# JohnGBaker/ptmcmc

Measured on AMD Instinct MI355X. Metric: ladder-wide MH steps/sec (D=32 Gaussian, 1024 temps), higher is better.
Workload: dtype f64

## Files before the change

### ptmcmc_amd/csrc/ptm_box_prefilter.hpp

```cpp
#pragma once
#include "ptm_kernels.hpp"

namespace ptm {

struct BoxPre {
  int W, Nt, r0, w_off;
  int rung0, nrung;
  int labelled;
  uint64_t seed, step;
  const double* x;
  const double *ll, *lp;
  const double* beta;
  const double* prop_tiles;
  const double* box_row;
  int* ntries;
  const int *pidx, *pcnt;
  int *cidx, *ccnt;
  unsigned long long* counts;
};

typedef double bp_d4 __attribute__((ext_vector_type(4)));
typedef double bp_d2 __attribute__((ext_vector_type(2)));

inline size_t box_prefilter_lds(int nrung) { return (size_t)(BM_TABLE_DOUBLES + 64) * sizeof(double) + ((size_t)nrung + 260) * sizeof(int); }

__global__ __launch_bounds__(256) void box_prefilter_kernel(const BoxPre p) {
  extern __shared__ __attribute__((aligned(16))) double bp_lds[];
  double* lbox = bp_lds + BM_TABLE_DOUBLES;
  int* tpre = reinterpret_cast<int*>(lbox + 64);
  const int wave = threadIdx.x >> 6, l = threadIdx.x & 63, q = l >> 4, j = l & 15;
#pragma unroll
  for (int t = 0; t < BM_TABLE_DOUBLES / 512; ++t)
    reinterpret_cast<bm_d2*>(bp_lds)[threadIdx.x + 256 * t] = reinterpret_cast<const bm_d2*>(BM_TABLE)[threadIdx.x + 256 * t];
  if (threadIdx.x < 64) lbox[threadIdx.x] = p.box_row[threadIdx.x];
  const int nrung = p.nrung, per = (nrung + 255) / 256;
  int loc = 0;
  for (int k = 0; k < per; ++k) {
    const int r = threadIdx.x * per + k;
    if (r < nrung) { loc += (p.pcnt[p.rung0 + r] + 255) >> 8; tpre[r] = loc; }
  }
  int* tsum = tpre + nrung;
  tsum[threadIdx.x] = loc;
  __syncthreads();
  if (threadIdx.x == 0) { int run = 0; for (int t = 0; t < 256; ++t) { const int v = tsum[t]; tsum[t] = run; run += v; } tsum[256] = run; }
  __syncthreads();
  const int off = tsum[threadIdx.x];
  for (int k = 0; k < per; ++k) {
    const int r = threadIdx.x * per + k;
    if (r < nrung) tpre[r] += off;
  }
  __syncthreads();
  const int ntiles = tsum[256];
  const bp_d2* box = reinterpret_cast<const bp_d2*>(lbox) + q;
  const int wmask = p.labelled ? 0xFFFF : -1;
  unsigned int seen = 0, settled = 0;
  for (int tile = blockIdx.x; tile < ntiles; tile += gridDim.x) {
    int lo = 0, hi = nrung - 1;
    while (lo < hi) { const int mid = (lo + hi) >> 1; if (tpre[mid] > tile) hi = mid; else lo = mid + 1; }
    const int r = __builtin_amdgcn_readfirstlane(lo);
    const int kb = tile - (r ? tpre[r - 1] : 0);
    const int rl = p.rung0 + r, rg = p.r0 + rl;
    const int start = (kb * 4 + wave) * 64, cnt = p.pcnt[rl];
    if (start >= cnt) continue;
    const int nact = cnt - start < 64 ? cnt - start : 64;
    const size_t lbase = (size_t)rl * p.W;
    const int mine = p.pidx[lbase + start + (l < nact ? l : nact - 1)];
    const int c = (int)lbase + (mine & wmask);
    const double ll = p.ll[c], lp = p.lp[c];
    const double beta = as_c(p.beta)[rg];
    const double* timg = p.prop_tiles + (size_t)rl * (16 * 64) + l;
    double ta[4];
#pragma unroll
    for (int sl = 0; sl < 4; ++sl) ta[sl] = timg[((0 * 4 + sl) * 2 + 0) * 64];
    const bp_d2 lo0 = box[0], lo1 = box[4], hi0 = box[16], hi1 = box[20];
    bp_d2 v0[4], v1[4];
    int wk[4];
#pragma unroll
    for (int g = 0; g < 4; ++g) {
      const int e = __shfl(mine, 16 * g + j, 64);
      const int slot = p.labelled ? (int)((unsigned int)e >> 16) : rl;
      wk[g] = e & wmask;
      const bp_d2* rp = reinterpret_cast<const bp_d2*>(p.x + ((size_t)slot * p.W + wk[g]) * 32) + q;
      v0[g] = rp[0];
      v1[g] = rp[4];
    }
    uint64_t inbox = 0;
#pragma unroll
    for (int g = 0; g < 4; ++g) {
      const uint32_t stream = (uint32_t)(wk[g] + p.w_off) * (uint32_t)p.Nt + (uint32_t)rg;
      const u32x4 o = draw_block(p.seed, TAG_MH, stream, p.step, (uint32_t)(1 + q));
      double z[4];
      boxmuller(o.v0, o.v1, (const double*)bp_lds, z[0], z[1]);
      boxmuller(o.v2, o.v3, (const double*)bp_lds, z[2], z[3]);
      bp_d4 acc = bp_d4{0.0, 0.0, 0.0, 0.0};
#pragma unroll
      for (int sl = 0; sl < 4; ++sl) acc = __builtin_amdgcn_mfma_f64_16x16x4f64(ta[sl], z[sl], acc, 0, 0, 0);
      const double x0 = v0[g].x + acc[0], x1 = v0[g].y + acc[1], x2 = v1[g].x + acc[2], x3 = v1[g].y + acc[3];
      const bool ok = !(x0 < lo0.x) & !(x0 > hi0.x) & !(x1 < lo0.y) & !(x1 > hi0.y) & !(x2 < lo1.x) & !(x2 > hi1.x) & !(x3 < lo1.y) & !(x3 > hi1.y);
      uint64_t b = __builtin_amdgcn_ballot_w64(ok);
      b &= b >> 32;
      b &= b >> 16;
      inbox |= (b & 0xFFFFull) << (16 * g);
    }
    const double cur_lpost = lp + beta * ll;
    const bool live = l < nact;
    const bool finite = __builtin_fabs(cur_lpost) < __builtin_inf();
    const bool settle = live && finite && ((inbox >> l) & 1ull) == 0;
    if (settle) p.ntries[c] += 1;
    const bool keep = live && !settle;
    const uint64_t kbits = __builtin_amdgcn_ballot_w64(keep);
    const int nk = __builtin_popcountll(kbits);
    int base = 0;
    if (l == 0 && nk) base = atomicAdd(&p.ccnt[rl], nk);
    base = __builtin_amdgcn_readfirstlane(base);
    if (keep) p.cidx[lbase + base + __builtin_popcountll(kbits & ((1ull << l) - 1ull))] = mine;
    seen += (unsigned int)nact;
    settled += (unsigned int)(nact - nk);
  }
  if (l == 0 && seen) {
    atomicAdd(p.counts, (unsigned long long)seen);
    if (settled) atomicAdd(p.counts + 1, (unsigned long long)settled);
  }
}

}
```

### ptmcmc_amd/csrc/ptm_engine.hip

```cpp
#include <hip/hip_runtime.h>

#include <algorithm>
#include <cmath>
#include <cstddef>
#include <cstdarg>
#include <cstdio>
#include <cstring>
#include <functional>
#include <memory>
#include <string>
#include <vector>

#include "../../include/ptm_engine.h"
#include "ptm_aux_kernels.hpp"
#include "ptm_box_prefilter.hpp"
#include "ptm_devlike_kernels.hpp"
#include "ptm_ess_kernels.hpp"
#include "ptm_evidence_kernels.hpp"
#include "ptm_launch.hpp"
#include "ptm_shard_rccl.hpp"

using namespace ptm;

static thread_local std::string g_err;
// ... 1145 lines not shown
  p.mix_K = e->mix_K; p.mix = e->mix;
  p.de_on = e->de_on ? 1 : 0; p.de_init_extra = e->de_init_extra; p.de_init = e->de_init; p.de_hast = e->de_hast; p.de_type = e->de_type;
  p.de_snooker = e->de.snooker; p.de_gamma_one = e->de.gamma_one_frac; p.de_gamma_div = e->de.reduce_gamma; p.de_ignore = e->de.ignore_frac;
  p.de_gamma_std = e->de_on ? 1.68 / std::sqrt((double)e->D) / e->de.reduce_gamma : 0.0;
  p.prior_k = e->prior_member + 1;
  p.betaC = e->betaC; p.beta_add = e->beta_add; p.beta_w = e->beta_w;
  p.x = labelled ? e->xdev : xrows(e); p.ll = e->ll; p.lp = e->lp;
  p.ntries = e->ntries; p.naccept = e->naccept; p.last_type = e->last_type; p.nhist = e->nhist;
  p.touch = e->touch; p.err = e->err;
  p.hist = e->hist;
  p.map = e->map;
  p.c_begin = 0; p.c_end = e->Nc;
  p.host_prop = e->pcb ? 1 : 0; p.hastings = e->hastings; p.htype = e->htype; p.hvalid = e->hvalid; p.acc_out = e->acc_out;
  return p;
}

static AdaArgs make_ada(const ptm_engine* e) {
  AdaArgs a;
  memset(&a, 0, sizeof a);
  if (!e->ada_on) return a;
  const size_t L = (size_t)e->ada.K + e->ada.K_inner, Nc = e->Nc;
  a.K = e->ada.K; a.nested = e->ada.nested; a.Ki = e->ada.K_inner; a.rate = e->ada.rate; a.rate_in = e->ada.rate_inner;
  a.leaf = e->ada_leaf; a.w = e->ada_dbl; a.th = e->ada_dbl + L * Nc; a.bits = e->ada_int; a.cnt = e->ada_int + 2 * Nc;
  return a;
}

const DpLaunch* ptm::dp_launch(int DP) {
  switch (DP) {
    case 4: return &dp_launch_4;
    case 8: return &dp_launch_8;
    case 16: return &dp_launch_16;
    case 32: return &dp_launch_32;
    case 64: return &dp_launch_64;
    case 128: return &dp_launch_128;
    case 256: return &dp_launch_256;
    case 512: return &dp_launch_512;
    case 1024: return &dp_launch_1024;
  }
  return nullptr;
}

static inline bool user_like(const ptm_engine* e) { return e->cb != nullptr || e->dfn != nullptr; }

static SweepPlan sweep_plan(const ptm_engine* e, long long chains, bool touched) {
  SweepFacts f;
  f.DP = e->DP; f.W = e->W; f.chains = chains; f.nloc = e->nloc;
  f.kind = e->prop_kind == PTM_PROP_DIAG ? PLAN_DIAG : (e->prop_kind == PTM_PROP_LOWER ? PLAN_LOWER : PLAN_DENSE);
  f.has_bounds = e->has_bounds; f.bounds_box = e->bounds_box; f.all_uniform = e->all_uniform; f.has_mean = e->has_mean; f.any_oned = e->any_oned;
  f.mix_K = e->mix_K;
  f.evolving = e->betaC != nullptr; f.tracked = e->hist.rungs || e->map.rungs;
  f.user_like = user_like(e); f.host_prop = e->pcb != nullptr; f.ada = e->ada_on;
  f.de = e->de_on || e->prior_member >= 0;
  f.mode = f.user_like ? 1 : 0;
  f.touched = touched;
  return plan_sweep(f, sweep_env());
}
static SweepPlan step_sweep_plan(const ptm_engine* e) { return sweep_plan(e, e->Nc, true); }

static bool lean_ev_sweeps(const ptm_engine* e) { return reads_ladder_major_beta(step_sweep_plan(e)); }

static int flush_nhist(ptm_engine* e) {
  if (!e->nhist_pending) return PTM_OK;
  hipLaunchKernelGGL(nhist_flush_kernel, dim3((unsigned)(((size_t)e->Nc + 255) / 256)), dim3(256), 0, e->stream, e->nhist, (size_t)e->Nc, e->nhist_pending);
  HIPCHK(hipGetLastError());
  e->nhist_pending = 0;
  return PTM_OK;
}

static bool row_labels_apply(const ptm_engine* e) {
  static const bool labels_ok = [] { const char* v = getenv("PTM_ROW_LABELS"); return !(v && *v == '0'); }();
  return labels_ok && e->nloc == e->Nt && !e->shard && e->W <= 65536 && e->Nt > 1 && step_sweep_plan(e).compacted;
}
static void flush_rows(ptm_engine* e) {
  e->rows_labelled = false;
  hipLaunchKernelGGL(restore_rows_kernel, dim3(e->W), dim3(256), (size_t)4 * e->nloc, e->stream, e->xdev, e->rowof, e->W, e->nloc, e->DP);
}

static int ensure_betaC(ptm_engine* e);
static int callback_host_part(ptm_engine* e) {
  const size_t Nc = e->Nc, DP = e->DP;
  HIPCHK(copy_unless_shared(e->h_xprop.data(), e->xprop, Nc * DP * 8 + Nc, hipMemcpyDeviceToHost, e->stream));
  HIPCHK(hipStreamSynchronize(e->stream));
  if (e->prior_cb) {
    std::vector<double> hll(Nc), hlp(Nc), hbeta(Nc), out;
    HIPCHK(hipMemcpy(hll.data(), e->ll, Nc * 8, hipMemcpyDeviceToHost));
    HIPCHK(hipMemcpy(hlp.data(), e->lp, Nc * 8, hipMemcpyDeviceToHost));
    { int rc2 = ensure_betaC(e); if (rc2) return rc2; }
    if (e->betaC) HIPCHK(hipMemcpy(hbeta.data(), e->betaC, Nc * 8, hipMemcpyDeviceToHost));
    std::vector<size_t> vp;
    for (size_t c = 0; c < Nc; ++c)
      if (e->h_gate[c] & 1) vp.push_back(c);
    int rcp = call_user_prior(e, e->h_xprop, vp, out);
    if (rcp) return rcp;
    std::vector<double> lpn(Nc, -__builtin_inf());
    for (size_t k = 0; k < vp.size(); ++k) {
      const size_t c = vp[k];
      const double beta = e->betaC ? hbeta[c] : e->h_beta[e->r0 + c / e->W];
      const double bl = beta * hll[c];
      const double cur_lpost = hlp[c] + bl;
      const double oldlprior = cur_lpost - bl;
      const double nl = out[k];
      lpn[c] = nl;
      const bool want = nl > -1e200 || nl - oldlprior > e->cfg.min_prior;
      e->h_gate[c] = (unsigned char)(1 | (want ? 2 : 0));
    }
    HIPCHK(hipMemcpyAsync(e->lprior_new, lpn.data(), Nc * 8, hipMemcpyHostToDevice, e->stream));
    HIPCHK(copy_unless_shared(e->gate, e->h_gate, Nc, hipMemcpyHostToDevice, e->stream));
    HIPCHK(hipStreamSynchronize(e->stream));
  }
  std::vector<size_t> pick;
  for (size_t c = 0; c < Nc; ++c)
    if (e->h_gate[c] & 2) pick.push_back(c);
  int rc = call_user(e, e->h_xprop, pick, e->h_llbatch);
  if (rc) return rc;
  for (size_t k = 0; k < pick.size(); ++k) e->h_llnew[pick[k]] = e->h_llbatch[k];
  HIPCHK(copy_unless_shared(e->llike_new, e->h_llnew.data(), Nc * 8, hipMemcpyHostToDevice, e->stream));
  return PTM_OK;
}

static int devlike_eval(ptm_engine* e, const unsigned char* gate, int gmask, int gval, const double* xsel, const double* xrest, double* dst,
                        unsigned char* gate_out, const double* lprior, bool best) {
  const int n = e->Nc, D = e->D;
  const int nchunk = (n + DL_CHUNK - 1) / DL_CHUNK;
  hipLaunchKernelGGL(devlike_count_kernel, dim3(nchunk), dim3(DL_CHUNK), 0, e->stream, n, gate, gmask, gval, e->dl_chunks);
  HIPCHK(hipGetLastError());
#define PTM_DL_PACK(N) case N: hipLaunchKernelGGL((devlike_pack_kernel<N>), dim3(nchunk), dim3(DL_CHUNK), 0, e->stream, n, D, nchunk, gate, gmask, gval, \
                                                  (const int*)e->dl_chunks, xsel, xrest, e->dl_x, e->dl_rows, e->dl_count); break;
  switch (e->DP) {
    PTM_DL_PACK(4) PTM_DL_PACK(8) PTM_DL_PACK(16) PTM_DL_PACK(32) PTM_DL_PACK(64) PTM_DL_PACK(128) PTM_DL_PACK(256) PTM_DL_PACK(512) PTM_DL_PACK(1024)
    default: return fail(PTM_ERR_UNSUPPORTED, "dim > 1024 is not built");
  }
#undef PTM_DL_PACK
  HIPCHK(hipGetLastError());
  if (!xrest) {
    const size_t tot = (size_t)n * D;
    hipLaunchKernelGGL(devlike_fill_kernel, dim3((unsigned)((tot + 255) / 256)), dim3(256), 0, e->stream, n, D, (const int32_t*)e->dl_count, e->dl_x);
    HIPCHK(hipGetLastError());
  }
  e->dfn(e->dfn_user, (void*)e->stream, n, D, e->dl_x, e->dl_count, e->dl_ll);
  hipLaunchKernelGGL(devlike_scatter_kernel, dim3(1), dim3(DL_SCATTER_THREADS), 0, e->stream, D, (const int32_t*)e->dl_count, (const int*)e->dl_rows,
                     (const double*)e->dl_ll, dst, gate_out, lprior, (const double*)e->dl_x, best ? e->dl_best : nullptr);
  HIPCHK(hipGetLastError());
  return PTM_OK;
}

static int devlike_reset_best(ptm_engine* e) {
  if (!e->dl_best) return PTM_OK;
  std::vector<double> b((size_t)e->D + 1, 0.0);
  b[0] = -__builtin_inf();
  return upload(e->dl_best, b.data(), b.size(), e->stream);
}

extern "C" int ptm_set_target_device(ptm_engine* e, ptm_loglike_device_fn fn, void* user, double* x_batch_dev, double* llike_batch_dev) {
  if (!e || !fn) return fail(PTM_ERR_INVALID, "null argument");
  SETTLE(e);
  NO_BATCH(e, "ptm_set_target_device");
  if (e->prior_cb) return fail(PTM_ERR_UNSUPPORTED, "a host-evaluated prior with a device likelihood is not built (ptm_set_prior_callback)");
  if (e->pcb) return fail(PTM_ERR_UNSUPPORTED, "host-side proposals with a device likelihood are not built (ptm_set_proposal_callback)");
  if (e->nloc != e->Nt) return fail(PTM_ERR_UNSUPPORTED, "a device likelihood on a rung shard is not built: split such a population by walkers");
  const size_t Nc = e->Nc, D = e->D, DP = e->DP;
  int rc;
  if (!e->dl_count &&
      ((rc = dalloc(&e->dl_count, 1)) || (rc = dalloc(&e->dl_rows, Nc)) || (rc = dalloc(&e->dl_chunks, (Nc + DL_CHUNK - 1) / DL_CHUNK)) ||
       (rc = dalloc(&e->dl_xprop, Nc * DP)) || (rc = dalloc(&e->dl_gate, Nc)) || (rc = dalloc(&e->dl_lprior_new, Nc)) ||
       (rc = dalloc(&e->dl_llike_new, Nc)) || (rc = dalloc(&e->dl_best, D + 1))))
    return rc;
  if (x_batch_dev) {
    if (e->dl_own_x && e->dl_x) { HIPCHK(hipStreamSynchronize(e->stream)); (void)hipFree(e->dl_x); }
    e->dl_x = x_batch_dev; e->dl_own_x = false;
  } else if (!e->dl_own_x) {
    e->dl_x = nullptr;
    if ((rc = dalloc(&e->dl_x, Nc * D))) return rc;
    e->dl_own_x = true;
  }
  if (llike_batch_dev) {
    if (e->dl_own_ll && e->dl_ll) { HIPCHK(hipStreamSynchronize(e->stream)); (void)hipFree(e->dl_ll); }
    e->dl_ll = llike_batch_dev; e->dl_own_ll = false;
  } else if (!e->dl_own_ll) {
    e->dl_ll = nullptr;
    if ((rc = dalloc(&e->dl_ll, Nc))) return rc;
    e->dl_own_ll = true;
  }
  HIPCHK(hipMemsetAsync(e->dl_gate, 0, Nc, e->stream));
  if ((rc = devlike_reset_best(e))) return rc;
  e->dfn = fn; e->dfn_user = user;
  e->cb = nullptr;
  e->have_target = 1;
  return PTM_OK;
}

extern "C" int ptm_target_device_rows(ptm_engine* e) {
  if (!e) return fail(PTM_ERR_INVALID, "null engine");
  return e->Nc;
}

extern "C" int ptm_get_best_evaluated(ptm_engine* e, double* lpost, double* x) {
  if (!e || !lpost) return fail(PTM_ERR_INVALID, "null argument");
  SETTLE(e);
  NO_BATCH(e, "ptm_get_best_evaluated");
  if (!e->dl_best) return fail(PTM_ERR_INVALID, "no device likelihood set (ptm_set_target_device)");
  std::vector<double> b((size_t)e->D + 1);
  HIPCHK(hipMemcpyAsync(b.data(), e->dl_best, b.size() * 8, hipMemcpyDeviceToHost, e->stream));
  HIPCHK(hipStreamSynchronize(e->stream));
  *lpost = b[0];
  if (x) memcpy(x, b.data() + 1, (size_t)e->D * 8);
  return PTM_OK;
}

static int devlike_debug(ptm_engine* e, const double* X, int n, double* llike) {
  const size_t Nc = e->Nc, D = e->D;
  std::vector<double> rows(Nc * D);
  for (size_t k0 = 0; k0 < (size_t)n; k0 += Nc) {
    const size_t m = std::min(Nc, (size_t)n - k0);
    for (size_t k = 0; k < Nc; ++k) memcpy(&rows[k * D], X + (k0 + (k < m ? k : 0)) * D, D * 8);
    const int32_t cnt = (int32_t)m;
    HIPCHK(hipMemcpyAsync(e->dl_x, rows.data(), Nc * D * 8, hipMemcpyHostToDevice, e->stream));
    HIPCHK(hipMemcpyAsync(e->dl_count, &cnt, 4, hipMemcpyHostToDevice, e->stream));
    e->dfn(e->dfn_user, (void*)e->stream, (int)Nc, (int)D, e->dl_x, e->dl_count, e->dl_ll);
    HIPCHK(hipMemcpyAsync(llike + k0, e->dl_ll, m * 8, hipMemcpyDeviceToHost, e->stream));
    HIPCHK(hipStreamSynchronize(e->stream));
  }
  return PTM_OK;
}

#define NO_DEVLIKE(e, name) do { if ((e) && (e)->dfn) return fail(PTM_ERR_UNSUPPORTED, name " with a device likelihood is not built (rung-sharded steps)"); } while (0)

static int prefilter_flags(ptm_engine* e) {
  const int nd = e->D < PREFILTER_DIMS ? e->D : PREFILTER_DIMS;
  double width[PREFILTER_DIMS];
  for (int d = 0; d < nd; ++d) width[d] = e->h_phi[d] - e->h_plo[d];
  if (!e->h_pf_flag) HIPCHK(hipHostMalloc((void**)&e->h_pf_flag, (size_t)e->nloc, hipHostMallocDefault));
  unsigned char* fl = e->h_pf_flag;
  e->pf_flagged = 0;
  for (int r = 0; r < e->nloc; ++r) {
    fl[r] = (e->pf_sigma.size() == (size_t)e->nloc * PREFILTER_DIMS && prefilter_flag(&e->pf_sigma[(size_t)r * PREFILTER_DIMS], width, nd, sweep_env().prefilter)) ? 1 : 0;
    e->pf_flagged += fl[r];
  }
  HIPCHK(hipMemcpyAsync(e->pf_flag, fl, (size_t)e->nloc, hipMemcpyHostToDevice, e->stream));
  e->pf_dirty = false;
  return PTM_OK;
}

static int launch_sweep(ptm_engine* e, int rung0 = 0, int nr = -1, bool last = true) {
  const bool labelled = e->label_step;
  e->label_step = false;
  Dev p = make_dev(e, labelled);
  if (nr < 0) nr = e->nloc - rung0;
  if (rung0 < 0 || nr < 0 || rung0 + nr > e->nloc) return fail(PTM_ERR_INVALID, "rung range out of the shard");
  p.c_begin = rung0 * e->W; p.c_end = (rung0 + nr) * e->W;
  if ((user_like(e) || e->pcb) && (rung0 != 0 || nr != e->nloc)) return fail(PTM_ERR_UNSUPPORTED, "partial sweeps with a user likelihood (host or device) or host-side proposals are not built");
  auto close_step = [&]() {
    e->step += 1; e->touched = false;
    if (e->compact_step) { e->nhist_pending += 1; e->compact_step = false; }
  };
  if (nr == 0) { if (last) close_step(); return PTM_OK; }
  hipEvent_t ev0 = nullptr, ev1 = nullptr;
  if (e->cfg.time_kernels) {
    if (e->kev_used + 2 > e->kev.size()) {
      for (int k = 0; k < 2; ++k) { hipEvent_t ev; HIPCHK(hipEventCreate(&ev)); e->kev.push_back(ev); }
    }
    ev0 = e->kev[e->kev_used]; ev1 = e->kev[e->kev_used + 1];
    e->kev_used += 2;
  }
  const SweepPlan plan = sweep_plan(e, p.c_end - p.c_begin, e->touched);
  if (e->betaC_stale && !reads_ladder_major_beta(plan)) { int rc = ensure_betaC(e); if (rc) return rc; }
  const bool compact = plan.compacted;
  if (labelled && !(compact && rung0 == 0 && nr == e->nloc)) return fail(PTM_ERR_HIP, "internal: a labelled exchange phase without its compacted sweep");
  if (!compact) { int rc = flush_nhist(e); if (rc) return rc; }
  if (compact) {
    if (!e->cidx) { int rc; if ((rc = dalloc(&e->cidx, (size_t)e->Nc)) || (rc = dalloc(&e->ccnt, (size_t)e->nloc))) return rc; }
    HIPCHK(hipMemsetAsync(e->ccnt + rung0, 0, (size_t)nr * sizeof(int), e->stream));
    bool pre = plan.prefilter;
    if (pre) {
      if (!e->pidx) {
        int rc;
        if ((rc = dalloc(&e->pidx, (size_t)e->Nc)) || (rc = dalloc(&e->pcnt, (size_t)e->nloc)) || (rc = dalloc(&e->pf_flag, (size_t)e->nloc)) || (rc = dalloc(&e->pf_counts, 2))) return rc;
        HIPCHK(hipMemsetAsync(e->pf_counts, 0, 16, e->stream));
        e->pf_dirty = true;
      }
      if (e->pf_dirty) { int rc = prefilter_flags(e); if (rc) return rc; }
      pre = e->pf_flagged > 0;
      if (pre) HIPCHK(hipMemsetAsync(e->pcnt + rung0, 0, (size_t)nr * sizeof(int), e->stream));
    }
    const int nchunk = (e->W + PART_CHUNK - 1) / PART_CHUNK;
    hipLaunchKernelGGL(partition_kernel, dim3((unsigned)((size_t)nr * nchunk)), dim3(1024), (size_t)PART_CHUNK * sizeof(int), e->stream, e->W, rung0, nchunk, e->touch, e->nhist,
                       e->cidx, e->ccnt, labelled ? (const unsigned short*)e->rowof : nullptr, pre ? (const unsigned char*)e->pf_flag : nullptr, e->pidx, e->pcnt);
    e->compact_step = true;
    HIPCHK(hipGetLastError());
    if (pre) {
      BoxPre b;
      memset(&b, 0, sizeof b);
      b.W = e->W; b.Nt = e->Nt; b.r0 = e->r0; b.w_off = e->cfg.walker_begin; b.rung0 = rung0; b.nrung = nr; b.labelled = labelled ? 1 : 0;
      b.seed = e->cfg.seed; b.step = e->step;
      b.x = p.x; b.ll = e->ll; b.lp = e->lp; b.beta = e->beta; b.prop_tiles = e->prop_tiles; b.box_row = e->box_row; b.ntries = e->ntries;
      b.pidx = e->pidx; b.pcnt = e->pcnt; b.cidx = e->cidx; b.ccnt = e->ccnt; b.counts = e->pf_counts;
      const size_t lds = box_prefilter_lds(nr);
      if (!e->pf_grid) {
        int per_cu = 0, dev = 0;
        hipDeviceProp_t pr;
        if (hipOccupancyMaxActiveBlocksPerMultiprocessor(&per_cu, (const void*)box_prefilter_kernel, 256, box_prefilter_lds(e->nloc)) != hipSuccess || per_cu <= 0) { (void)hipGetLastError(); per_cu = 2; }
        HIPCHK(hipGetDevice(&dev));
        HIPCHK(hipGetDeviceProperties(&pr, dev));
        e->pf_grid = per_cu * (pr.multiProcessorCount > 0 ? pr.multiProcessorCount : 256);
      }
      const long long tiles = (long long)nr * ((e->W + 255) / 256);
      hipLaunchKernelGGL(box_prefilter_kernel, dim3((unsigned)(tiles < e->pf_grid ? tiles : e->pf_grid)), dim3(256), lds, e->stream, b);
      HIPCHK(hipGetLastError());
    }
    p.cidx = e->cidx; p.ccnt = e->ccnt; p.cidx_slot = labelled ? 1 : 0;
  }
  if (ev0) HIPCHK(hipEventRecord(ev0, e->stream));
  const AdaArgs ada = make_ada(e);
  const DpLaunch* dl = dp_launch(e->DP);
  if (!dl) return fail(PTM_ERR_UNSUPPORTED, "dim > 1024 is not built");
  auto launch = [&](const Dev& q) { return dl->sweep(q, plan, e->stream, ada); };

  size_t npick = 0;
  if (e->pcb) {
    const size_t Nc = e->Nc, D = e->D, DP = e->DP;
    HIPCHK(hipMemcpyAsync(e->h_rows.data(), xrows(e), Nc * DP * 8, hipMemcpyDeviceToHost, e->stream));
    HIPCHK(hipMemcpyAsync(e->h_touch.data(), e->touch, Nc, hipMemcpyDeviceToHost, e->stream));
    HIPCHK(hipStreamSynchronize(e->stream));
    e->p_pick.clear();
    for (size_t c = 0; c < Nc; ++c)
      if (!e->h_touch[c]) e->p_pick.push_back(c);
    npick = e->p_pick.size();
    e->p_xcur.resize(npick * D); e->p_xprop.assign(npick * D, 0.0); e->p_hast.assign(npick, 0.0);
    e->p_rung.resize(npick); e->p_walker.resize(npick); e->p_type.assign(npick, 0); e->p_valid.assign(npick, 1);
    for (size_t k = 0; k < npick; ++k) {
      const size_t c = e->p_pick[k];
      for (size_t d = 0; d < D; ++d) e->p_xcur[k * D + d] = e->h_rows[c * DP + host_row_pos(DP, d)];
      e->p_rung[k] = e->r0 + (int)(c / e->W); e->p_walker[k] = e->cfg.walker_begin + (int)(c % e->W);
    }
    if (npick)
      e->pcb(e->pcb_user, (int)npick, (int)D, e->p_xcur.data(), e->p_rung.data(), e->p_walker.data(), e->step, e->p_xprop.data(),
             e->p_hast.data(), e->p_type.data(), e->p_valid.data());
    for (size_t k = 0; k < npick; ++k) {
      const size_t c = e->p_pick[k];
      for (size_t d = 0; d < DP; ++d) e->h_xprop[c * DP + d] = 0.0;
      for (size_t d = 0; d < D; ++d) e->h_xprop[c * DP + host_row_pos(DP, d)] = e->p_xprop[k * D + d];
      e->h_hast[c] = e->p_hast[k]; e->h_type[c] = e->p_type[k]; e->h_valid[c] = e->p_valid[k] ? 1 : 0;
    }
    HIPCHK(copy_unless_shared(e->xprop, e->h_xprop.data(), Nc * DP * 8, hipMemcpyHostToDevice, e->stream));
    HIPCHK(copy_unless_shared(e->hastings, e->h_hast.data(), Nc * 8, hipMemcpyHostToDevice, e->stream));
    HIPCHK(copy_unless_shared(e->htype, e->h_type.data(), Nc * 4, hipMemcpyHostToDevice, e->stream));
    HIPCHK(copy_unless_shared(e->hvalid, e->h_valid.data(), Nc, hipMemcpyHostToDevice, e->stream));
    p.xprop = e->xprop; p.lprior_new = e->lprior_new; p.gate = e->gate; p.llike_new = e->llike_new;
  }
  if (e->dfn) {
    p.xprop = e->dl_xprop; p.lprior_new = e->dl_lprior_new; p.gate = e->dl_gate; p.llike_new = e->dl_llike_new;
    p.mode = 1;
    HIPCHK(launch(p));
    { const int rc = devlike_eval(e, e->dl_gate, 2, 2, e->dl_xprop, xrows(e), e->dl_llike_new, nullptr, e->dl_lprior_new, true); if (rc) return rc; }
    p.mode = 2;
    HIPCHK(launch(p));
  } else if (!e->cb) {
    HIPCHK(launch(p));
  } else {
    const size_t Nc = e->Nc, DP = e->DP;
    p.xprop = e->xprop; p.lprior_new = e->lprior_new; p.gate = e->gate; p.llike_new = e->llike_new;
    p.mode = 1;
    HIPCHK(launch(p));
    { const int rc = callback_host_part(e); if (rc) return rc; }
    p.mode = 2;
    HIPCHK(launch(p));
  }
  if (e->pcb && e->pres && npick) {
    HIPCHK(copy_unless_shared(e->h_acc.data(), e->acc_out, (size_t)e->Nc, hipMemcpyDeviceToHost, e->stream));
    HIPCHK(hipStreamSynchronize(e->stream));
    e->p_acc.resize(npick);
    for (size_t k = 0; k < npick; ++k) e->p_acc[k] = e->h_acc[e->p_pick[k]] == 1 ? 1 : 0;
    e->pres(e->pcb_user, (int)npick, e->p_rung.data(), e->p_walker.data(), e->p_acc.data());
  }
  if (ev1) HIPCHK(hipEventRecord(ev1, e->stream));
  if (last) close_step();
  return PTM_OK;
}

static int fold_swap_log(ptm_engine* e) {
  if (!e->log_pending) return PTM_OK;
  const int first = ((e->log_head - e->log_pending) % PTM_LOG_RING + PTM_LOG_RING) % PTM_LOG_RING;
  if (e->Nt > 1) {
    hipLaunchKernelGGL(fold_swap_log_kernel, dim3(e->W), dim3(256), (size_t)2 * (e->Nt - 1) * sizeof(int), e->stream, e->swap_log, e->swap_cnt,
                       e->W, e->ms, e->Nt, e->r0, e->r0 + e->nloc, first, e->log_pending);
    HIPCHK(hipGetLastError());
  }
  e->log_pending = 0;
  return PTM_OK;
}

static int launch_beta_transpose(ptm_engine* e) {
  e->betaC_stale = false;
  if (e->nloc != e->Nt) {
    hipLaunchKernelGGL(beta_local_kernel, dim3((unsigned)(((size_t)e->Nc + 255) / 256)), dim3(256), 0, e->stream, e->beta_w, e->betaC, e->W, e->Nt, e->r0, e->nloc);
    HIPCHK(hipGetLastError());
    return PTM_OK;
  }
  hipLaunchKernelGGL(beta_transpose_kernel, dim3((e->Nt + 31) / 32, (e->W + 31) / 32), dim3(256), 0, e->stream, e->beta_w, e->betaC, e->W, e->Nt);
  HIPCHK(hipGetLastError());
  return PTM_OK;
}
static int ensure_betaC(ptm_engine* e) {
  if (!e->betaC_stale) return PTM_OK;
  e->betaC_stale = false;
  return launch_beta_transpose(e);
}

static Decide make_decide(ptm_engine* e, const double* ll_below, const double* ll_above, int H, double* send_up, double* send_down,
                          const double* ll_all = nullptr, const double* lp_all = nullptr, bool labels = false) {
  Decide p;
  memset(&p, 0, sizeof p);
  p.rowof = labels ? e->rowof : nullptr;
  p.ll_all = ll_all; p.lp_all = lp_all;
  p.shard_ends = e->shard_ends; p.nshards = e->nshards; p.halo_nominal = e->halo_nominal;
  p.redo_flag = e->redo_flag; p.redo_count = e->redo_flag ? e->redo_flag + e->W : nullptr;
  p.DP = e->DP; p.Nt = e->Nt; p.r0 = e->r0; p.nloc = e->nloc; p.W = e->W; p.Nc = e->Nc; p.ms = e->ms; p.w_off = e->cfg.walker_begin;
  p.seed = e->cfg.seed; p.step = e->step; p.thresh = e->thresh;
  p.beta = e->beta; p.ll_below = ll_below; p.ll_above = ll_above; p.H = ll_above ? H : 0; p.x = labels ? e->xdev : xrows(e); p.ll = e->ll; p.lp = e->lp;
  p.touch = e->touch; p.arr_below = e->arr_below; p.arr_above = e->arr_above;
  p.swap_log = e->swap_log + (size_t)e->log_head * e->W * e->ms; p.send_up = send_up; p.send_down = send_down; p.row_cap = e->row_cap; p.err = e->err;
  p.mv_src = e->mv_src; p.mv_dst = e->mv_dst; p.mv_n = e->mv_n;
  p.hist = e->hist; p.add_every_n = e->cfg.add_every_n; p.nhist = e->nhist;
  p.naccept = e->naccept; p.ntries = e->ntries; p.last_type = e->last_type;
  p.map = e->map;
  p.evolve_rate = e->evolve_rate; p.evolve_cut = e->evolve_cut; p.beta_w = e->beta_w; p.beta_add = e->beta_add;
  p.lp_is_const = e->lp_is_const ? 1 : 0; p.lp_const = e->lprior_const;
  static const bool direct_all = [] { const char* v = getenv("PTM_BETA_DIRECT"); return v && *v == '1'; }();
  const bool beta_direct = e->evolve_rate > 0 && (e->W <= 64 || direct_all);
  p.betaC_direct = beta_direct ? e->betaC : nullptr;
  return p;
}

static int launch_decide(ptm_engine* e, const double* ll_below, const double* ll_above, int H, double* send_up, double* send_down,
                         const double* ll_all = nullptr, const double* lp_all = nullptr, bool redo = false, bool labels = false) {
  if (labels && !e->rowof) {
    int rc = dalloc(&e->rowof, (size_t)e->Nc);
    if (rc) return rc;
    hipLaunchKernelGGL(identity_rows_kernel, dim3((unsigned)(((size_t)e->Nc + 255) / 256)), dim3(256), 0, e->stream, e->rowof, e->W, (size_t)e->Nc);
    HIPCHK(hipGetLastError());
  }
  Decide p = make_decide(e, ll_below, ll_above, H, send_up, send_down, ll_all, lp_all, labels);
  if (labels) { e->rows_labelled = true; e->label_step = true; }
  p.redo_only = redo ? 1 : 0;
  if (!redo && e->log_pending >= PTM_LOG_RING) { int rc = fold_swap_log(e); if (rc) return rc; }
  if (redo) {
    const int slot = (e->log_head + PTM_LOG_RING - 1) % PTM_LOG_RING;
    p.swap_log = e->swap_log + (size_t)slot * e->W * e->ms;
  }
  const bool beta_direct = p.betaC_direct != nullptr;
  e->touched = true;
  const int WN = ll_all ? e->Nt : e->nloc + (ll_below ? 1 : 0) + p.H;
  const bool evb = e->evolve_rate > 0 && e->beta_add;
  const bool cut = e->evolve_rate > 0 && e->evolve_cut >= 0;
  const size_t lds = decide_lds_bytes(e->Nt, e->ms, WN, e->evolve_rate > 0, evb, cut);
  if (lds > 160 * 1024) return fail(PTM_ERR_UNSUPPORTED, "ladder too long for the LDS-resident exchange kernel (%zu B)", lds);
  if (e->ms >= 65535) return fail(PTM_ERR_UNSUPPORTED, "more than 65534 exchange candidates per step (the exchange kernel numbers them in 16 bits)");
  const int per_pick = (e->nloc == e->Nt ? 2 : 4) + (e->hist.rungs ? 1 : 0) + (e->map.rungs ? 1 : 0);
  const bool wide = (double)e->ms * WN / e->Nt > 96.0 || evb || cut || (e->W <= 256 && per_pick * e->ms > 64);
  if (lds > 64 * 1024) {
    HIPCHK(hipFuncSetAttribute((const void*)decide_kernel<64>, hipFuncAttributeMaxDynamicSharedMemorySize, (int)lds));
    HIPCHK(hipFuncSetAttribute((const void*)decide_kernel<256>, hipFuncAttributeMaxDynamicSharedMemorySize, (int)lds));
  }
  if (send_up && !redo) HIPCHK(hipMemsetAsync(send_up, 0, 16, e->stream));
  if (send_down && !redo) HIPCHK(hipMemsetAsync(send_down, 0, 16, e->stream));
  if (cut) {
    if (lds > 64 * 1024) HIPCHK(hipFuncSetAttribute((const void*)decide_kernel<256, true>, hipFuncAttributeMaxDynamicSharedMemorySize, (int)lds));
    hipLaunchKernelGGL((decide_kernel<256, true>), dim3(e->W), dim3(256), lds, e->stream, p);
  } else if (wide) hipLaunchKernelGGL(decide_kernel<256>, dim3(e->W), dim3(256), lds, e->stream, p);
  else hipLaunchKernelGGL(decide_kernel<64>, dim3(e->W), dim3(64), lds, e->stream, p);
  HIPCHK(hipGetLastError());
  if (!redo) {
    e->log_head = (e->log_head + 1) % PTM_LOG_RING;
    ++e->log_pending;
  }
  if (e->evolve_rate > 0 && !beta_direct) {
    if (lean_ev_sweeps(e)) e->betaC_stale = true;
    else { e->betaC_stale = false; int rc = launch_beta_transpose(e); if (rc) return rc; }
  }
  if (wide) return PTM_OK;
  if (per_pick * e->ms <= 64 || labels) return PTM_OK;
  Move m;
  m.DP = e->DP; m.W = e->W; m.row_cap = e->row_cap; m.x = xrows(e); m.ll = e->ll; m.lp = e->lp; m.send_up = send_up; m.send_down = send_down;
  m.mv_src = e->mv_src; m.mv_dst = e->mv_dst; m.mv_n = e->mv_n; m.err = e->err;
  m.hist = e->hist; m.add_every_n = e->cfg.add_every_n; m.nhist = e->nhist;
  m.naccept = e->naccept; m.ntries = e->ntries; m.last_type = e->last_type;
  m.map = e->map; m.beta = e->beta; m.r0 = e->r0;
  const dim3 mgrid((unsigned)((e->W + 63) / 64));
  if (e->hist.rungs || e->map.rungs) hipLaunchKernelGGL((move_kernel<MVCAP, 1, true>), mgrid, dim3(64), 0, e->stream, m);
  else hipLaunchKernelGGL((move_kernel<MVCAP, 1, false>), mgrid, dim3(64), 0, e->stream, m);
  HIPCHK(hipGetLastError());
  return PTM_OK;
}

static int launch_install(ptm_engine* e, const double* recv_below, const double* recv_above) {
  if (!recv_below && !recv_above) return PTM_OK;
  Install q;
  q.DP = e->DP; q.W = e->W; q.row_cap = e->row_cap; q.x = xrows(e); q.ll = e->ll; q.lp = e->lp;
  q.recv_below = recv_below; q.recv_above = recv_above; q.arr_below = e->arr_below; q.arr_above = e->arr_above; q.err = e->err;
  e->touched = true;
  hipLaunchKernelGGL(install_kernel, dim3((e->row_cap + 15) / 16, 2), dim3(256), 0, e->stream, q);
  HIPCHK(hipGetLastError());
  return PTM_OK;
}

static int ready(ptm_engine* e) {
  if (!e) return fail(PTM_ERR_INVALID, "null engine");
  if (!e->have_target) return fail(PTM_ERR_INVALID, "no target set (ptm_set_target_gaussian)");
  if (!e->have_ladder) return fail(PTM_ERR_INVALID, "no ladder set (ptm_set_ladder)");
  if (!e->have_prop) return fail(PTM_ERR_INVALID, "no proposals set (ptm_set_proposals)");
  if (!e->have_state) return fail(PTM_ERR_INVALID, "no states set (ptm_set_states / ptm_init_from_prior)");
  if (e->prior_member >= 0) return prior_drawable(e);
  return PTM_OK;
}

static int check_lp_const(ptm_engine* e) {
  e->lp_is_const = false;
  if (!e->all_uniform || e->prior_cb) return PTM_OK;
  std::vector<double> lp((size_t)e->Nc);
  HIPCHK(hipStreamSynchronize(e->stream));
  HIPCHK(hipMemcpy(lp.data(), e->lp, lp.size() * 8, hipMemcpyDeviceToHost));
  for (double v : lp)
    if (!(v == e->lprior_const)) return PTM_OK;
  e->lp_is_const = true;
  return PTM_OK;
}
static int reset_counters(ptm_engine* e) {
  const size_t Nc = e->Nc;
  std::vector<int> one(Nc, 1), m1(Nc, -1);
  std::vector<unsigned int> z(Nc, 0u);
  int rc;
  if ((rc = upload(e->ntries, one.data(), Nc, e->stream)) || (rc = upload(e->naccept, one.data(), Nc, e->stream)) ||
      (rc = upload(e->last_type, m1.data(), Nc, e->stream)) ||
      (rc = upload(e->nhist, z.data(), Nc, e->stream)))
    return rc;
  e->nhist_pending = 0; e->compact_step = false; e->touched = false;
  HIPCHK(hipMemsetAsync(e->touch, 0, Nc, e->stream));
  HIPCHK(hipMemsetAsync(e->arr_below, 0xFF, (size_t)e->W * 4, e->stream));
  HIPCHK(hipMemsetAsync(e->arr_above, 0xFF, (size_t)e->W * 4, e->stream));
  e->step = 0;
  if (e->map.rungs) {
    if (!e->have_ladder) return fail(PTM_ERR_INVALID, "set the ladder before the states when tracking the MAP (ptm_set_ladder)");
    hipLaunchKernelGGL(map_init_kernel, dim3((e->map.MC + 255) / 256), dim3(256), 0, e->stream, e->map, e->DP, e->W, e->r0, e->beta, xrows(e), e->ll,
                       e->lp);
    HIPCHK(hipGetLastError());
  }
  if (e->hist.rungs) {
    HIPCHK(hipMemsetAsync(e->hist.meta, 0xFF, (size_t)e->hist.cap * e->hist.HC * sizeof(int4), e->stream));
    if (e->hist.beta && !e->have_ladder) return fail(PTM_ERR_INVALID, "set the ladder before the states (ptm_set_ladder)");
    hipLaunchKernelGGL(hist_init_kernel, dim3((e->hist.HC + 255) / 256), dim3(256), 0, e->stream, e->hist, e->DP, xrows(e), e->ll, e->lp,
                       e->naccept, e->ntries, e->last_type, e->beta, e->betaC, e->W, e->r0);
    HIPCHK(hipGetLastError());
  }
  return PTM_OK;
}

static int run_eval(ptm_engine* e, int n, double* x, int* valid, double* lp, double* ll, int eval_like) {
  Dev p = make_dev(e);
  const DpLaunch* dl = dp_launch(e->DP);
  if (!dl) return fail(PTM_ERR_UNSUPPORTED, "dim > 1024 is not built");
  HIPCHK(dl->eval(p, n, x, valid, lp, ll, eval_like, e->stream));
  return PTM_OK;
}

static inline size_t host_row_pos(size_t DP, size_t d) { return (DP == 32 || DP == 64 || DP == 128) ? 8 * ((d >> 2) >> 1) + 2 * (d & 3) + ((d >> 2) & 1) : d; }
static std::vector<double> pad_rows(const double* X, size_t n, size_t D, size_t DP) {
  std::vector<double> r(n * DP, 0.0);
  for (size_t c = 0; c < n; ++c)
    for (size_t d = 0; d < D; ++d) r[c * DP + host_row_pos(DP, d)] = X[c * D + d];
  return r;
}
static void unpad_rows(const double* r, size_t n, size_t D, size_t DP, double* X) {
  for (size_t c = 0; c < n; ++c)
    for (size_t d = 0; d < D; ++d) X[c * D + d] = r[c * DP + host_row_pos(DP, d)];
}
static void unpad_rows(const std::vector<double>& r, size_t n, size_t D, size_t DP, double* X) { unpad_rows(r.data(), n, D, DP, X); }

extern "C" int ptm_set_states(ptm_engine* e, const double* X, const double* llike) {
  SETTLE(e);
  NO_BATCH(e, "ptm_set_states");
  if (!e || !X) return fail(PTM_ERR_INVALID, "null argument");
  if (!e->have_target && !llike) return fail(PTM_ERR_INVALID, "set the target first (or pass llike)");
  const size_t Nc = e->Nc, D = e->D, DP = e->DP;
  const std::vector<double> rows = pad_rows(X, Nc, D, DP);
  int rc;
  if ((rc = upload(xrows(e), rows.data(), Nc * DP, e->stream))) return rc;
  if (llike && (rc = upload(e->ll, llike, Nc, e->stream))) return rc;
  if ((rc = run_eval(e, (int)Nc, xrows(e), nullptr, e->lp, e->ll, (llike || user_like(e)) ? 0 : 1))) return rc;
  if (e->dfn) {
    if ((rc = devlike_reset_best(e))) return rc;
    if (!llike && (rc = devlike_eval(e, nullptr, 0, 0, xrows(e), xrows(e), e->ll, nullptr, e->lp, true))) return rc;
  }
  if (e->cb && !llike) {
    HIPCHK(hipStreamSynchronize(e->stream));
    HIPCHK(hipMemcpy(e->h_xprop.data(), xrows(e), Nc * DP * 8, hipMemcpyDeviceToHost));
    std::vector<size_t> all(Nc);
    for (size_t c = 0; c < Nc; ++c) all[c] = c;
    if ((rc = call_user(e, e->h_xprop, all, e->h_llbatch))) return rc;
    if ((rc = upload(e->ll, e->h_llbatch.data(), Nc, e->stream))) return rc;
  }
  if (e->prior_cb) {
    if (!e->cb) return fail(PTM_ERR_UNSUPPORTED, "a host-evaluated prior needs the host-callback likelihood (ptm_set_target_callback)");
    HIPCHK(hipStreamSynchronize(e->stream));
    HIPCHK(hipMemcpy(e->h_xprop.data(), xrows(e), Nc * DP * 8, hipMemcpyDeviceToHost));
    if ((rc = host_prior_of_states(e))) return rc;
  }
  if ((rc = reset_counters(e))) return rc;
// ... 1576 lines not shown
```

### ptmcmc_amd/csrc/ptm_sweep_plan.hpp

```cpp
#pragma once
#include <cmath>
#include <cstddef>
#include <cstdio>
#include <cstdlib>

namespace ptm {

enum { PLAN_DENSE = 0, PLAN_DIAG = 1, PLAN_LOWER = 2 };

struct SweepFacts {
  int DP, W;
  long long chains;
  int nloc;
  int kind;
  bool has_bounds, bounds_box, all_uniform, has_mean, any_oned;
  int mix_K;
  bool evolving;
  bool tracked;
  bool user_like;
  bool host_prop;
  bool de, ada;
  int mode;
  bool touched;
};

struct SweepEnv {
  bool force_valu, compact_ok;
  int prefilter;
};
inline const SweepEnv& sweep_env() {
  static const SweepEnv v = [] {
    const char* f = getenv("PTM_FORCE_VALU");
    const char* c = getenv("PTM_COMPACT");
    const char* b = getenv("PTM_BOX_PREFILTER");
    return SweepEnv{f && *f && *f != '0', !(c && *c == '0'), (b && *b) ? (*b == '0' ? -1 : 1) : 0};
  }();
  return v;
}

enum SweepFamily { FAM_GENERAL, FAM_LANES, FAM_LANES_ADA, FAM_MFMA32, FAM_MFMA64, FAM_MFMA128 };

struct SweepPlan {
  SweepFamily family;
  int DP, kind;
  bool uni, simple, ada;
  bool gen;
  bool hist;
  int mgen;
  bool ev;
  bool bnd;
  bool compacted;
  bool prefilter;
};
inline bool reads_ladder_major_beta(const SweepPlan& s) { return s.family == FAM_MFMA32 && s.mgen == 0 && s.ev; }

#define PTM_LANES_MAX (1ll << 20)

inline SweepPlan plan_sweep(const SweepFacts& f, const SweepEnv& env) {
  SweepPlan s = {};
  s.DP = f.DP;
  s.kind = f.host_prop ? PLAN_DIAG : f.kind;
  const bool uni = (f.W % 64) == 0;
  const bool ada = f.ada && !f.host_prop;
  const bool box = f.all_uniform && (!f.has_bounds || f.bounds_box);
  const bool recipe = f.has_mean || f.any_oned || f.mix_K != 0;
  const bool plain = !f.has_bounds && f.all_uniform && !recipe && !f.user_like && !ada && !f.evolving && !f.host_prop;
  const bool simple = uni && plain;
  const bool lean_ev = uni && f.evolving && !f.has_bounds && f.all_uniform && !recipe && !f.user_like && !ada && !f.host_prop && !f.tracked;
  const bool mfma_ok = uni && f.mode == 0 && !f.user_like && !f.host_prop && !ada && !env.force_valu;
  const int mk = s.kind == PLAN_DIAG ? PLAN_LOWER : s.kind;

  if (f.DP == 32 && mfma_ok && !f.de) {
    s.family = FAM_MFMA32; s.kind = mk;
    s.compacted = env.compact_ok && f.touched && box && !f.tracked && f.W >= 1024 && f.nloc <= 4096;
    s.hist = f.tracked;
    s.mgen = (simple || lean_ev) ? 0 : !box ? 2 : (s.compacted && !recipe) ? 3 : 1;
    s.ev = !simple && box && f.evolving;
    s.prefilter = env.prefilter >= 0 && s.compacted && s.mgen == 0 && !s.ev && (f.kind == PLAN_LOWER || f.kind == PLAN_DIAG);
    return s;
  }
  if ((f.DP == 64 || f.DP == 128) && mfma_ok && box && !recipe && !f.tracked) {
    s.family = f.DP == 64 ? FAM_MFMA64 : FAM_MFMA128; s.kind = mk;
    s.bnd = f.has_bounds; s.ev = f.evolving;
    return s;
  }
  const long long lanes = f.chains * f.DP;
  const long long lanes_max = f.DP >= 16 ? PTM_LANES_MAX : 4096ll * f.DP, lanes_max_de = f.DP >= 32 ? (1ll << 21) : (1ll << 19);
  if (f.DP >= 64 || f.host_prop ||
      (!env.force_valu && ((!uni && lanes <= lanes_max) || (uni && f.de && f.DP >= 16 && lanes <= lanes_max_de)))) {
    s.family = ada ? FAM_LANES_ADA : FAM_LANES;
    s.gen = !plain;
    return s;
  }
  s.family = FAM_GENERAL;
  s.uni = uni; s.simple = simple; s.ada = ada;
  return s;
}

constexpr int PREFILTER_DIMS = 16;
#ifndef PTM_PREFILTER_THRESHOLD
#define PTM_PREFILTER_THRESHOLD 0.70
#endif
inline void prefilter_sigmas(bool diag, const double* factor, int D, double* sigma) {
  for (int d = 0; d < PREFILTER_DIMS; ++d) {
    double s2 = 0.0;
    if (d < D) {
      if (diag) s2 = factor[d] * factor[d];
      else for (int k = 0; k < D; ++k) s2 += factor[(size_t)d * D + k] * factor[(size_t)d * D + k];
    }
    sigma[d] = std::sqrt(s2);
  }
}
inline double prefilter_out_1d(double sigma, double w) {
  if (!(sigma > 0.0) || !(w < INFINITY)) return 0.0;
  if (!(w > 0.0)) return 1.0;
  const double u = w / sigma, phi0 = 0.3989422804014327;
  const double in = std::erf(u * 0.7071067811865476) - (2.0 / u) * (phi0 - phi0 * std::exp(-0.5 * u * u));
  return in < 0.0 ? 1.0 : (in > 1.0 ? 0.0 : 1.0 - in);
}
inline double prefilter_out_share(const double* sigma, const double* width, int nd) {
  double in = 1.0;
  for (int d = 0; d < nd; ++d) in *= 1.0 - prefilter_out_1d(sigma[d], width[d]);
  return 1.0 - in;
}
inline bool prefilter_flag(const double* sigma, const double* width, int nd, int env_prefilter) {
  if (env_prefilter < 0) return false;
  if (env_prefilter > 0) return true;
  return prefilter_out_share(sigma, width, nd) > PTM_PREFILTER_THRESHOLD;
}

inline int format_sweep_name(const SweepPlan& s, char* b, size_t n) {
  const auto tf = [](bool v) { return v ? "true" : "false"; };
  switch (s.family) {
    case FAM_MFMA32: return snprintf(b, n, "sweep_mfma32_kernel<%d, %s, %d, %s, %s>", s.kind, tf(s.hist), s.mgen, tf(s.ev), tf(s.compacted));
    case FAM_MFMA64:
    case FAM_MFMA128: return snprintf(b, n, "sweep_mfma%d_kernel<%d, %s, %s>", s.DP, s.kind, tf(s.bnd), tf(s.ev));
    case FAM_LANES: return snprintf(b, n, "sweep_lanes_kernel<%d, %d, %s>", s.DP, s.kind, tf(s.gen));
    case FAM_LANES_ADA: return snprintf(b, n, "sweep_lanes_ada_kernel<%d, %d>", s.DP, s.kind);
    default: break;
  }
  if (s.ada) return snprintf(b, n, "sweep_kernel<%d, %d, %s, false, true>", s.DP, s.kind, tf(s.uni));
  return snprintf(b, n, "sweep_kernel<%d, %d, %s, %s>", s.DP, s.kind, tf(s.uni), tf(s.simple));
}

struct StepFacts {
  int DP, Nt, W;
  bool user_like, host_prop, ada, time_kernels;
  bool evolving, evolve_cut;
  size_t decide_lds;
};
inline bool fused_applies(const StepFacts& f, bool fused_ok) {
  if (!fused_ok || f.DP > 16 || (long long)f.Nt * f.DP > 256 || f.user_like || f.host_prop || f.ada || f.time_kernels) return false;
  if (f.evolving && (f.W > 64 || f.evolve_cut)) return false;
  return f.decide_lds <= 96 * 1024;
}

}
```

Before: 10.87 billion.

## Software-pipeline box prefilter tiles with lookahead index loads and deferred compaction writes

Restructures the prefilter loop so the next tile's slice lookup and pidx entry load are issued one iteration ahead, with an optional two-deep row prefetch behind a compile flag (off by default). Rung counts are cached in LDS, the cidx scatter is deferred to the next iteration so the ccnt atomic latency overlaps compute, and ntries becomes a relaxed atomic. Launch bounds now request a minimum occupancy, and an env var can cap the grid. The aim is to hide global-load and atomic latency in a memory-bound filter, at the cost of extra registers, sched barriers and more complex control flow.

Measured after the change: 11.48 billion (median of 6 runs). 5.7% higher.

```diff
diff --git a/ptmcmc_amd/csrc/ptm_box_prefilter.hpp b/ptmcmc_amd/csrc/ptm_box_prefilter.hpp
--- a/ptmcmc_amd/csrc/ptm_box_prefilter.hpp
+++ b/ptmcmc_amd/csrc/ptm_box_prefilter.hpp
@@ -1,7 +1,12 @@
 #pragma once
 #include "ptm_kernels.hpp"
+#include "ptm_sweep_plan.hpp"
 
 namespace ptm {
+
+#ifndef PTM_BP_ROWS_AHEAD
+#define PTM_BP_ROWS_AHEAD 0
+#endif
 
 struct BoxPre {
   int W, Nt, r0, w_off;
@@ -22,9 +27,16 @@
 typedef double bp_d4 __attribute__((ext_vector_type(4)));
 typedef double bp_d2 __attribute__((ext_vector_type(2)));
 
-inline size_t box_prefilter_lds(int nrung) { return (size_t)(BM_TABLE_DOUBLES + 64) * sizeof(double) + ((size_t)nrung + 260) * sizeof(int); }
+#define PTM_BP_STAGE() __builtin_amdgcn_sched_barrier(0)
 
-__global__ __launch_bounds__(256) void box_prefilter_kernel(const BoxPre p) {
+struct BpRows {
+  bp_d2 v0[4], v1[4];
+  double ll, lp, beta, ta[4];
+};
+
+inline size_t box_prefilter_lds(int nrung) { return (size_t)(BM_TABLE_DOUBLES + 64) * sizeof(double) + (2 * (size_t)nrung + 260) * sizeof(int); }
+
+__global__ __launch_bounds__(256, PTM_BP_ROWS_AHEAD ? 3 : 4) void box_prefilter_kernel(const BoxPre p) {
   extern __shared__ __attribute__((aligned(16))) double bp_lds[];
   double* lbox = bp_lds + BM_TABLE_DOUBLES;
   int* tpre = reinterpret_cast<int*>(lbox + 64);
@@ -34,12 +46,13 @@
     reinterpret_cast<bm_d2*>(bp_lds)[threadIdx.x + 256 * t] = reinterpret_cast<const bm_d2*>(BM_TABLE)[threadIdx.x + 256 * t];
   if (threadIdx.x < 64) lbox[threadIdx.x] = p.box_row[threadIdx.x];
   const int nrung = p.nrung, per = (nrung + 255) / 256;
+  int* pcn = tpre + nrung;
   int loc = 0;
   for (int k = 0; k < per; ++k) {
     const int r = threadIdx.x * per + k;
-    if (r < nrung) { loc += (p.pcnt[p.rung0 + r] + 255) >> 8; tpre[r] = loc; }
+    if (r < nrung) { const int n = p.pcnt[p.rung0 + r]; pcn[r] = n; loc += (n + 255) >> 8; tpre[r] = loc; }
   }
-  int* tsum = tpre + nrung;
+  int* tsum = pcn + nrung;
   tsum[threadIdx.x] = loc;
   __syncthreads();
   if (threadIdx.x == 0) { int run = 0; for (int t = 0; t < 256; ++t) { const int v = tsum[t]; tsum[t] = run; run += v; } tsum[256] = run; }
@@ -53,70 +66,117 @@
   const int ntiles = tsum[256];
   const bp_d2* box = reinterpret_cast<const bp_d2*>(lbox) + q;
   const int wmask = p.labelled ? 0xFFFF : -1;
-  unsigned int seen = 0, settled = 0;
-  for (int tile = blockIdx.x; tile < ntiles; tile += gridDim.x) {
-    int lo = 0, hi = nrung - 1;
-    while (lo < hi) { const int mid = (lo + hi) >> 1; if (tpre[mid] > tile) hi = mid; else lo = mid + 1; }
-    const int r = __builtin_amdgcn_readfirstlane(lo);
-    const int kb = tile - (r ? tpre[r - 1] : 0);
-    const int rl = p.rung0 + r, rg = p.r0 + rl;
-    const int start = (kb * 4 + wave) * 64, cnt = p.pcnt[rl];
-    if (start >= cnt) continue;
-    const int nact = cnt - start < 64 ? cnt - start : 64;
-    const size_t lbase = (size_t)rl * p.W;
-    const int mine = p.pidx[lbase + start + (l < nact ? l : nact - 1)];
-    const int c = (int)lbase + (mine & wmask);
-    const double ll = p.ll[c], lp = p.lp[c];
-    const double beta = as_c(p.beta)[rg];
+  const int G = (int)gridDim.x;
+
+  auto slice_of = [&](int tile) {
+    PrefilterSlice s = prefilter_slice(tpre, pcn, nrung, ntiles, tile, wave);
+    s.r = __builtin_amdgcn_readfirstlane(s.r);
+    s.start = __builtin_amdgcn_readfirstlane(s.start);
+    s.nact = __builtin_amdgcn_readfirstlane(s.nact);
+    return s;
+  };
+  auto load_entry = [&](const PrefilterSlice& s) {
+    if (s.nact == 0) return 0;
+    return p.pidx[(size_t)(p.rung0 + s.r) * p.W + s.start + (l < s.nact ? l : s.nact - 1)];
+  };
+  auto load_rows = [&](const PrefilterSlice& s, int mine, BpRows& R) {
+    if (s.nact == 0) return;
+    const int rl = p.rung0 + s.r;
+    const int c = (int)((size_t)rl * p.W) + (mine & wmask);
+    R.ll = p.ll[c]; R.lp = p.lp[c];
+    R.beta = as_c(p.beta)[p.r0 + rl];
     const double* timg = p.prop_tiles + (size_t)rl * (16 * 64) + l;
-    double ta[4];
 #pragma unroll
-    for (int sl = 0; sl < 4; ++sl) ta[sl] = timg[((0 * 4 + sl) * 2 + 0) * 64];
-    const bp_d2 lo0 = box[0], lo1 = box[4], hi0 = box[16], hi1 = box[20];
-    bp_d2 v0[4], v1[4];
-    int wk[4];
+    for (int sl = 0; sl < 4; ++sl) R.ta[sl] = timg[((0 * 4 + sl) * 2 + 0) * 64];
 #pragma unroll
     for (int g = 0; g < 4; ++g) {
       const int e = __shfl(mine, 16 * g + j, 64);
       const int slot = p.labelled ? (int)((unsigned int)e >> 16) : rl;
-      wk[g] = e & wmask;
-      const bp_d2* rp = reinterpret_cast<const bp_d2*>(p.x + ((size_t)slot * p.W + wk[g]) * 32) + q;
-      v0[g] = rp[0];
-      v1[g] = rp[4];
+      const bp_d2* rp = reinterpret_cast<const bp_d2*>(p.x + ((size_t)slot * p.W + (e & wmask)) * 32) + q;
+      R.v0[g] = rp[0];
+      R.v1[g] = rp[4];
     }
+  };
+
+  constexpr bool RA = PTM_BP_ROWS_AHEAD != 0;
+  constexpr int EA = RA ? 2 : 1;
+  PrefilterSlice sl[EA + 1] = {};
+  int m[EA + 1] = {};
+  BpRows R[2] = {};
+#pragma unroll
+  for (int k = 0; k < EA; ++k) { sl[k] = slice_of((int)blockIdx.x + k * G); m[k] = load_entry(sl[k]); }
+  if (RA) load_rows(sl[0], m[0], R[0]);
+  uint64_t pbits = 0;
+  int pmine = 0, pbase = 0;
+  size_t plbase = 0;
+  auto flush = [&]() {
+    if (pbits == 0) return;
+    const int base = __builtin_amdgcn_readfirstlane(pbase);
+    if ((pbits >> l) & 1ull) p.cidx[plbase + base + __builtin_popcountll(pbits & ((1ull << l) - 1ull))] = pmine;
+    pbits = 0;
+  };
+#define PTM_BP_ARRIVED() __builtin_amdgcn_s_waitcnt(0x0F70)
+  PTM_BP_ARRIVED();
+  unsigned int seen = 0, settled = 0;
+  for (int tile = blockIdx.x; tile < ntiles; tile += G) {
+    sl[EA] = slice_of(tile + EA * G);
+    m[EA] = load_entry(sl[EA]);
+    if (RA) load_rows(sl[1], m[1], R[1]);
+    else load_rows(sl[0], m[0], R[0]);
+    PTM_BP_STAGE();
+    const PrefilterSlice s = sl[0];
+    const int mine = m[0], nact = s.nact;
+    const int rl = p.rung0 + s.r, rg = p.r0 + rl;
+    const size_t lbase = (size_t)rl * p.W;
+    const BpRows& T = R[0];
     uint64_t inbox = 0;
+    if (nact) {
+      const bp_d2 lo0 = box[0], lo1 = box[4], hi0 = box[16], hi1 = box[20];
 #pragma unroll
-    for (int g = 0; g < 4; ++g) {
-      const uint32_t stream = (uint32_t)(wk[g] + p.w_off) * (uint32_t)p.Nt + (uint32_t)rg;
-      const u32x4 o = draw_block(p.seed, TAG_MH, stream, p.step, (uint32_t)(1 + q));
-      double z[4];
-      boxmuller(o.v0, o.v1, (const double*)bp_lds, z[0], z[1]);
-      boxmuller(o.v2, o.v3, (const double*)bp_lds, z[2], z[3]);
-      bp_d4 acc = bp_d4{0.0, 0.0, 0.0, 0.0};
+      for (int g = 0; g < 4; ++g) {
+        const int wk = __shfl(mine, 16 * g + j, 64) & wmask;
+        const uint32_t stream = (uint32_t)(wk + p.w_off) * (uint32_t)p.Nt + (uint32_t)rg;
+        const u32x4 o = draw_block(p.seed, TAG_MH, stream, p.step, (uint32_t)(1 + q));
+        double z[4];
+        boxmuller(o.v0, o.v1, (const double*)bp_lds, z[0], z[1]);
+        boxmuller(o.v2, o.v3, (const double*)bp_lds, z[2], z[3]);
+        bp_d4 acc = bp_d4{0.0, 0.0, 0.0, 0.0};
 #pragma unroll
-      for (int sl = 0; sl < 4; ++sl) acc = __builtin_amdgcn_mfma_f64_16x16x4f64(ta[sl], z[sl], acc, 0, 0, 0);
-      const double x0 = v0[g].x + acc[0], x1 = v0[g].y + acc[1], x2 = v1[g].x + acc[2], x3 = v1[g].y + acc[3];
-      const bool ok = !(x0 < lo0.x) & !(x0 > hi0.x) & !(x1 < lo0.y) & !(x1 > hi0.y) & !(x2 < lo1.x) & !(x2 > hi1.x) & !(x3 < lo1.y) & !(x3 > hi1.y);
-      uint64_t b = __builtin_amdgcn_ballot_w64(ok);
-      b &= b >> 32;
-      b &= b >> 16;
-      inbox |= (b & 0xFFFFull) << (16 * g);
+        for (int k = 0; k < 4; ++k) acc = __builtin_amdgcn_mfma_f64_16x16x4f64(T.ta[k], z[k], acc, 0, 0, 0);
+        const double x0 = T.v0[g].x + acc[0], x1 = T.v0[g].y + acc[1], x2 = T.v1[g].x + acc[2], x3 = T.v1[g].y + acc[3];
+        const bool ok = !(x0 < lo0.x) & !(x0 > hi0.x) & !(x1 < lo0.y) & !(x1 > hi0.y) & !(x2 < lo1.x) & !(x2 > hi1.x) & !(x3 < lo1.y) & !(x3 > hi1.y);
+        uint64_t b = __builtin_amdgcn_ballot_w64(ok);
+        b &= b >> 32;
+        b &= b >> 16;
+        inbox |= (b & 0xFFFFull) << (16 * g);
+      }
     }
-    const double cur_lpost = lp + beta * ll;
-    const bool live = l < nact;
-    const bool finite = __builtin_fabs(cur_lpost) < __builtin_inf();
-    const bool settle = live && finite && ((inbox >> l) & 1ull) == 0;
-    if (settle) p.ntries[c] += 1;
-    const bool keep = live && !settle;
-    const uint64_t kbits = __builtin_amdgcn_ballot_w64(keep);
-    const int nk = __builtin_popcountll(kbits);
-    int base = 0;
-    if (l == 0 && nk) base = atomicAdd(&p.ccnt[rl], nk);
-    base = __builtin_amdgcn_readfirstlane(base);
-    if (keep) p.cidx[lbase + base + __builtin_popcountll(kbits & ((1ull << l) - 1ull))] = mine;
-    seen += (unsigned int)nact;
-    settled += (unsigned int)(nact - nk);
+    PTM_BP_STAGE();
+    PTM_BP_ARRIVED();
+    if (nact) {
+      const int c = (int)lbase + (mine & wmask);
+      const double cur_lpost = T.lp + T.beta * T.ll;
+      const bool live = l < nact;
+      const bool finite = __builtin_fabs(cur_lpost) < __builtin_inf();
+      const bool settle = live && finite && ((inbox >> l) & 1ull) == 0;
+      const bool keep = live && !settle;
+      const uint64_t kbits = __builtin_amdgcn_ballot_w64(keep);
+      const int nk = __builtin_popcountll(kbits);
+      flush();
+      if (settle) (void)__hip_atomic_fetch_add(&p.ntries[c], 1, __ATOMIC_RELAXED, __HIP_MEMORY_SCOPE_AGENT);
+      if (nk) {
+        pbits = kbits; pmine = mine; plbase = lbase;
+        const int rlv = __builtin_amdgcn_mov_dpp(rl, 0xE4, 0xF, 0xF, true);
+        if (l == 0) pbase = atomicAdd(&p.ccnt[rlv], nk);
+      }
+      seen += (unsigned int)nact;
+      settled += (unsigned int)(nact - nk);
+    }
+#pragma unroll
+    for (int k = 0; k < EA; ++k) { sl[k] = sl[k + 1]; m[k] = m[k + 1]; }
+    if (RA) R[0] = R[1];
   }
+  flush();
   if (l == 0 && seen) {
     atomicAdd(p.counts, (unsigned long long)seen);
     if (settled) atomicAdd(p.counts + 1, (unsigned long long)settled);
diff --git a/ptmcmc_amd/csrc/ptm_engine.hip b/ptmcmc_amd/csrc/ptm_engine.hip
--- a/ptmcmc_amd/csrc/ptm_engine.hip
+++ b/ptmcmc_amd/csrc/ptm_engine.hip
@@ -1471,6 +1471,8 @@
         HIPCHK(hipGetDevice(&dev));
         HIPCHK(hipGetDeviceProperties(&pr, dev));
         e->pf_grid = per_cu * (pr.multiProcessorCount > 0 ? pr.multiProcessorCount : 256);
+        const int cap = sweep_env().prefilter_grid;
+        if (cap > 0 && cap < e->pf_grid) e->pf_grid = cap;
       }
       const long long tiles = (long long)nr * ((e->W + 255) / 256);
       hipLaunchKernelGGL(box_prefilter_kernel, dim3((unsigned)(tiles < e->pf_grid ? tiles : e->pf_grid)), dim3(256), lds, e->stream, b);
diff --git a/ptmcmc_amd/csrc/ptm_sweep_plan.hpp b/ptmcmc_amd/csrc/ptm_sweep_plan.hpp
--- a/ptmcmc_amd/csrc/ptm_sweep_plan.hpp
+++ b/ptmcmc_amd/csrc/ptm_sweep_plan.hpp
@@ -27,13 +27,16 @@
 struct SweepEnv {
   bool force_valu, compact_ok;
   int prefilter;
+  int prefilter_grid;
 };
 inline const SweepEnv& sweep_env() {
   static const SweepEnv v = [] {
     const char* f = getenv("PTM_FORCE_VALU");
     const char* c = getenv("PTM_COMPACT");
     const char* b = getenv("PTM_BOX_PREFILTER");
-    return SweepEnv{f && *f && *f != '0', !(c && *c == '0'), (b && *b) ? (*b == '0' ? -1 : 1) : 0};
+    const char* g = getenv("PTM_PREFILTER_GRID");
+    const long gn = (g && *g) ? strtol(g, nullptr, 10) : 0;
+    return SweepEnv{f && *f && *f != '0', !(c && *c == '0'), (b && *b) ? (*b == '0' ? -1 : 1) : 0, gn >= 1 ? (int)(gn < (1 << 20) ? gn : (1 << 20)) : 0};
   }();
   return v;
 }
@@ -129,6 +132,25 @@
   return prefilter_out_share(sigma, width, nd) > PTM_PREFILTER_THRESHOLD;
 }
 
+#ifdef __HIPCC__
+#define PTM_PLAN_HD __host__ __device__
+#else
+#define PTM_PLAN_HD
+#endif
+struct PrefilterSlice { int r, kb, start, nact; };
+PTM_PLAN_HD inline PrefilterSlice prefilter_slice(const int* tpre, const int* cnt, int nrung, int ntiles, int tile, int wave) {
+  PrefilterSlice s = {0, 0, 0, 0};
+  if (tile < 0 || tile >= ntiles) return s;
+  int lo = 0, hi = nrung - 1;
+  while (lo < hi) { const int mid = (lo + hi) >> 1; if (tpre[mid] > tile) hi = mid; else lo = mid + 1; }
+  s.r = lo;
+  s.kb = tile - (lo ? tpre[lo - 1] : 0);
+  s.start = (s.kb * 4 + wave) * 64;
+  const int left = cnt[lo] - s.start;
+  s.nact = left <= 0 ? 0 : (left < 64 ? left : 64);
+  return s;
+}
+
 inline int format_sweep_name(const SweepPlan& s, char* b, size_t n) {
   const auto tf = [](bool v) { return v ? "true" : "false"; };
   switch (s.family) {
```
